# ysymyth/3D-SDN

Hardware: AMD Instinct MI355X
Metric: rendered-objects/sec (FFD decode + transform + silhouette/normal/depth @384, fwd+bwd) (higher is better)
Workload: dtype f32

## Files before the change

### 3d-sdn_amd/csrc/raster_fwd.hip

```cpp
#include <mutex>
#include <type_traits>
#include <vector>

#include "camera_math.h"
#include "raster_math.h"
#include "sdn_common.h"

namespace sdn {

constexpr int TS = 32;
constexpr int NTHR = (TS / 2) * (TS / 2);
constexpr int NWAVE = NTHR / 64;
static_assert(NTHR % 64 == 0 && NTHR >= 2 * TS && TS <= 32, "tile / workgroup geometry (hit queue packs px, py in 5 bits)");
constexpr int QCAP = 512;
constexpr int FREC = 13;
#ifndef SDN_LAB_FLAT_MAX
#define SDN_LAB_FLAT_MAX 256
#endif
constexpr int FLAT_MAX = SDN_LAB_FLAT_MAX;
static_assert(FLAT_MAX >= 1 && FLAT_MAX <= 256, "a batch's stream holds at most 64 * 256 candidates: 14 bits of start, at most 256 passes (the marks are u16, 0xffff = none)");
#ifndef SDN_LAB_HIZ_MIN_LIST
#define SDN_LAB_HIZ_MIN_LIST 257
#endif
constexpr int HIZ_MIN_LIST = SDN_LAB_HIZ_MIN_LIST;
#ifndef SDN_K1_HIZ
#define SDN_K1_HIZ 1
#endif
constexpr uint32_t TB_CULLED = 0x000000FFu;

struct FwdParams {
    const float* faces;
    const float* textures;
    const float* bg;
    float* face_inv;
    int32_t* face_index_map;
    float* weight_map;
    float* depth_map;
    float* rgb_map;
    float* rgb_out;
    float* alpha_out;
    float* depth_out;
    const uint32_t* tilebox;
    const uint4* pixbox;
    const uint32_t* tile_off;
    const uint32_t* tile_list;
    const uint32_t* overflow;
    const uint32_t* tile_order;
    const uint32_t* thin_count;
    const float4* thin_list;
    unsigned long long* counters;
    uint32_t list_cap;
    double eps;
    int ts, bs, nf, S, ntx, flags, bg_per_batch;
    int hiz;
    float near_le, far_f;
};

constexpr float THIN_MARGIN = 4.0f;

__device__ __forceinline__ float face_margin_px(const float f[9], int S)
{
    const float ex0 = f[3] - f[0], ey0 = f[4] - f[1];
    const float ex1 = f[6] - f[0], ey1 = f[7] - f[1];
    const float ex2 = f[6] - f[3], ey2 = f[7] - f[4];
    const float l0 = sqrtf(ex0 * ex0 + ey0 * ey0);
    const float l1 = sqrtf(ex1 * ex1 + ey1 * ey1);
    const float l2 = sqrtf(ex2 * ex2 + ey2 * ey2);
    const float lmax = fmaxf(l0, fmaxf(l1, l2));
    const float perim = l0 + l1 + l2;
    float cmax = fmaxf(fmaxf(fabsf(f[0]), fabsf(f[1])), fmaxf(fabsf(f[3]), fabsf(f[4])));
    cmax = fmaxf(cmax, fmaxf(fabsf(f[6]), fabsf(f[7])));
    const float area2 = fabsf(ex0 * ey1 - ex1 * ey0) - 9.5367432e-7f * lmax * lmax;
    if (!(area2 > 0.0f)) return -1.0f;
    const float delta = 9.5367432e-7f * (1.0f + cmax);
    const float base = 0.004f * fmaxf(1.0f, (float)S * (1.0f / 1024.0f)) + 0.5f * (float)S * delta;
    const float m = base + 0.5f * (float)S * (delta * perim * lmax / area2);
    if (!(m < (float)S)) return -1.0f;
    return m;
}

constexpr int HIST_MAX = 4096;

template <bool K1, bool GATHER>
__global__ __launch_bounds__(256) void k_face_setup(const float* __restrict__ faces, int nf, int S, int ntx,
                                                     float* __restrict__ face_inv, uint32_t* __restrict__ tilebox,
                                                     uint4* __restrict__ pixbox, uint32_t* __restrict__ tile_count,
                                                     uint32_t* __restrict__ thin_count, float4* __restrict__ thin_list,
                                                     const FaceSource G)
{
    __shared__ uint32_t hist[HIST_MAX];
    const int ntiles = ntx * ntx;
    const bool use_lds = ntiles <= HIST_MAX;
    if (use_lds)
        for (int t = threadIdx.x; t < ntiles; t += 256) hist[t] = 0u;
    __syncthreads();
    const int b = blockIdx.y;
    const int t_local = blockIdx.x * 256 + threadIdx.x;
    uint32_t* gcount = tile_count + (size_t)b * ntiles;
    const bool pairs = GATHER && G.fill_back != 0;
    const int nthr = pairs ? G.nf0 : nf;
    float v[3][3], pf[9];
    if constexpr (GATHER) {
        if (t_local < nthr) {
            const int32_t* idx = G.faces_idx + (size_t)b * G.fstride + (size_t)t_local * 3;
#pragma unroll
            for (int k = 0; k < 3; k++) {
                const float* p = G.verts + ((size_t)b * G.nv + idx[k]) * 3;
                v[k][0] = G.flip_x ? p[0] * -1.0f : p[0];
                v[k][1] = p[1];
                v[k][2] = p[2];
            }
            Basis B;
            if (G.mode != 0) B = camera_basis(G.mode, G.eye, G.dir, G.up, b);
            const float wv = G.width ? G.width[b] : 1.0f;
#pragma unroll
            for (int k = 0; k < 3; k++) {
                float o[3];
                project_vertex(v[k], G.mode, B, G.width != nullptr, wv, o);
                pf[3 * k + 0] = o[0];
                pf[3 * k + 1] = o[1];
                pf[3 * k + 2] = o[2];
            }
        }
    }
    if (t_local < nthr)
    for (int rep = 0; rep < (pairs ? 2 : 1); rep++) {
    const int fn_local = t_local + (rep ? G.nf0 : 0);
    const long i = (long)b * nf + fn_local;
    float f[9];
    float nrm[3] = {0.f, 0.f, 0.f};
    if constexpr (GATHER) {
        if (G.normals_out) {
            if (rep)
                face_normal(v[2], v[1], v[0], G.sx, nrm);
            else
                face_normal(v[0], v[1], v[2], G.sx, nrm);
        }
#pragma unroll
        for (int k = 0; k < 3; k++)
#pragma unroll
            for (int d = 0; d < 3; d++) f[3 * k + d] = rep ? pf[3 * (2 - k) + d] : pf[3 * k + d];
    } else {
#pragma unroll
        for (int k = 0; k < 9; k++) f[k] = faces[i * 9 + k];
    }
    float inv[9] = {0, 0, 0, 0, 0, 0, 0, 0, 0};
    uint32_t tb = TB_CULLED;
    uint4 pb = make_uint4(0, 0, 0, 0);
    bool thin = false;
    if constexpr (K1) {
      if (!is_backface(f)) {
        bool finite = true;
#pragma unroll
        for (int k = 0; k < 9; k++) finite = finite && (f[k] - f[k] == 0.0f);
        const K1Face K = k1_setup(f, S);
        if (finite && !K.dead && K.xi_min <= K.xi_max) {
            float inv_s[9];
            face_inverse(K.px, K.py, inv_s);
#pragma unroll
            for (int l = 0; l < 3; l++)
#pragma unroll
                for (int k = 0; k < 3; k++) {
                    const float v = inv_s[3 * l + k];
                    if (K.pi[l] == 0) inv[k] = v;
                    if (K.pi[l] == 1) inv[3 + k] = v;
                    if (K.pi[l] == 2) inv[6 + k] = v;
                }
            const float ymin = fminf(K.py[0], fminf(K.py[1], K.py[2])), ymax = fmaxf(K.py[0], fmaxf(K.py[1], K.py[2]));
            int y0 = 0, y1 = S - 1;
            if (!(K.px[2] < 0.0f)) {
                y0 = (int)fmaxf(floorf(ymin) - 1.0f, 0.0f);
                y1 = (int)fminf(ceilf(ymax) + 1.0f, (float)(S - 1));
            }
            if (y0 <= y1 && ymax + 1.0f >= 0.0f && ymin - 1.0f <= (float)(S - 1)) {
                const int x0 = K.xi_min, x1 = K.xi_max;
                tb = (uint32_t)(x0 / TS) | ((uint32_t)(x1 / TS) << 8) | ((uint32_t)(y0 / TS) << 16) | ((uint32_t)(y1 / TS) << 24);
                pb = make_uint4((uint32_t)x0 | ((uint32_t)x1 << 16), (uint32_t)y0 | ((uint32_t)y1 << 16), 0u, 0u);
                for (int ty = y0 / TS; ty <= y1 / TS; ty++)
                    for (int tx = x0 / TS; tx <= x1 / TS; tx++) {
                        if (use_lds)
                            atomicAdd(&hist[ty * ntx + tx], 1u);
                        else
                            atomicAdd(&gcount[ty * ntx + tx], 1u);
                    }
            }
        }
      }
    } else if (!is_backface(f)) {
        const float is_f = (float)S;
        float px[3], py[3];
#pragma unroll
        for (int k = 0; k < 3; k++) {
            px[k] = ndc_to_pixel(f[3 * k + 0], is_f);
            py[k] = ndc_to_pixel(f[3 * k + 1], is_f);
        }
        face_inverse(px, py, inv);
        int x0 = 0, x1 = S - 1, y0 = 0, y1 = S - 1;
        const float m = face_margin_px(f, S);
        const float xmin = fminf(px[0], fminf(px[1], px[2])), xmax = fmaxf(px[0], fmaxf(px[1], px[2]));
        const float ymin = fminf(py[0], fminf(py[1], py[2])), ymax = fmaxf(py[0], fmaxf(py[1], py[2]));
        const bool finite = (xmin - xmin == 0.0f) && (xmax - xmax == 0.0f) && (ymin - ymin == 0.0f) &&
                            (ymax - ymax == 0.0f) && (px[0] == px[0]) && (px[1] == px[1]) && (px[2] == px[2]) &&
                            (py[0] == py[0]) && (py[1] == py[1]) && (py[2] == py[2]);
        bool visible = true;
        if (!finite) {
            visible = false;
        } else if (!(m > 0.0f) || m > THIN_MARGIN) {
            visible = false;
            int ia = 0, ib = 1;
            float l2 = (px[1] - px[0]) * (px[1] - px[0]) + (py[1] - py[0]) * (py[1] - py[0]);
            const float l2b = (px[2] - px[0]) * (px[2] - px[0]) + (py[2] - py[0]) * (py[2] - py[0]);
            const float l2c = (px[2] - px[1]) * (px[2] - px[1]) + (py[2] - py[1]) * (py[2] - py[1]);
            if (l2b > l2) { l2 = l2b; ia = 0; ib = 2; }
            if (l2c > l2) { l2 = l2c; ia = 1; ib = 2; }
            if (l2 > 0.0f) {
                const float L = sqrtf(l2);
                const float nx = -(py[ib] - py[ia]) / L, ny = (px[ib] - px[ia]) / L;
                const int ic = 3 - ia - ib;
                const float h = fabsf((px[ic] - px[ia]) * nx + (py[ic] - py[ia]) * ny);
                const float pmax = fmaxf(fmaxf(fabsf(xmin), fabsf(xmax)), fmaxf(fabsf(ymin), fabsf(ymax)));
                float cmax = fmaxf(fmaxf(fabsf(f[0]), fabsf(f[1])), fmaxf(fabsf(f[3]), fabsf(f[4])));
                cmax = fmaxf(cmax, fmaxf(fabsf(f[6]), fabsf(f[7])));
                const float delta_px = 9.5367432e-7f * (1.0f + cmax) * 0.5f * (float)S;
                const float band = h + 0.05f + 2.5f * delta_px + 4e-6f * (pmax + (float)S);
                const bool repeated = (__float_as_uint(f[0]) == __float_as_uint(f[3]) && __float_as_uint(f[1]) == __float_as_uint(f[4])) ||
                                      (__float_as_uint(f[0]) == __float_as_uint(f[6]) && __float_as_uint(f[1]) == __float_as_uint(f[7])) ||
                                      (__float_as_uint(f[3]) == __float_as_uint(f[6]) && __float_as_uint(f[4]) == __float_as_uint(f[7]));
                int bx0 = 0, bx1 = S - 1, by0 = 0, by1 = S - 1;
                bool boxed_out = false;
                if (m > 0.0f) {
                    const float fx0 = ceilf(xmin - m), fx1 = floorf(xmax + m);
                    const float fy0 = ceilf(ymin - m), fy1 = floorf(ymax + m);
                    if (fx1 < 0.0f || fy1 < 0.0f || fx0 > (float)(S - 1) || fy0 > (float)(S - 1) || fx0 > fx1 || fy0 > fy1) {
                        boxed_out = true;
                    } else {
                        bx0 = (int)fmaxf(fx0, 0.0f);
                        by0 = (int)fmaxf(fy0, 0.0f);
                        bx1 = (int)fminf(fx1, (float)(S - 1));
                        by1 = (int)fminf(fy1, (float)(S - 1));
                    }
                }
                if (!(repeated && band < 0.5f) && !boxed_out) {
                    const uint32_t trange = (uint32_t)(bx0 / TS) | ((uint32_t)(bx1 / TS) << 8) | ((uint32_t)(by0 / TS) << 16) |
                                            ((uint32_t)(by1 / TS) << 24);
                    pb = make_uint4((uint32_t)bx0 | ((uint32_t)bx1 << 16), (uint32_t)by0 | ((uint32_t)by1 << 16), __float_as_uint(m), 0u);
                    const uint32_t slot = atomicAdd(&thin_count[b], 1u);
                    float4* e = thin_list + (size_t)b * nf * 2;
                    e[slot] = make_float4(nx, ny, px[ia] * nx + py[ia] * ny, band);
                    e[nf + slot] = make_float4(px[ia], py[ia], __uint_as_float((uint32_t)fn_local), __uint_as_float(trange));
                    thin = true;
                }
            }
        } else {
            const float fx0 = ceilf(xmin - m), fx1 = floorf(xmax + m);
            const float fy0 = ceilf(ymin - m), fy1 = floorf(ymax + m);
            if (fx1 < 0.0f || fy1 < 0.0f || fx0 > (float)(S - 1) || fy0 > (float)(S - 1) || fx0 > fx1 || fy0 > fy1) {
                visible = false;
            } else {
                x0 = (int)fmaxf(fx0, 0.0f);
                y0 = (int)fmaxf(fy0, 0.0f);
                x1 = (int)fminf(fx1, (float)(S - 1));
                y1 = (int)fminf(fy1, (float)(S - 1));
            }
        }
        if (visible) {
            tb = (uint32_t)(x0 / TS) | ((uint32_t)(x1 / TS) << 8) | ((uint32_t)(y0 / TS) << 16) |
                 ((uint32_t)(y1 / TS) << 24);
            pb = make_uint4((uint32_t)x0 | ((uint32_t)x1 << 16), (uint32_t)y0 | ((uint32_t)y1 << 16), __float_as_uint(m), 0u);
            for (int ty = y0 / TS; ty <= y1 / TS; ty++)
                for (int tx = x0 / TS; tx <= x1 / TS; tx++) {
                    if (use_lds)
                        atomicAdd(&hist[ty * ntx + tx], 1u);
                    else
                        atomicAdd(&gcount[ty * ntx + tx], 1u);
                }
        }
    }
    tilebox[i] = tb;
    if (!GATHER || tb != TB_CULLED || thin) {
#pragma unroll
        for (int k = 0; k < 9; k++) face_inv[i * 9 + k] = inv[k];
        pixbox[i] = pb;
        if constexpr (GATHER) {
            float* fo = G.faces_out + i * 9;
#pragma unroll
            for (int k = 0; k < 9; k++) fo[k] = f[k];
            if (G.normals_out) {
                float* o = G.normals_out + i * 3;
                o[0] = nrm[0];
                o[1] = nrm[1];
                o[2] = nrm[2];
            }
        }
    }
    }
    __syncthreads();
    if (use_lds)
        for (int t = threadIdx.x; t < ntiles; t += 256) {
            const uint32_t c = hist[t];
            if (c) atomicAdd(&gcount[t], c);
        }
}

constexpr int ORDER_CLASSES = 64;
__device__ __forceinline__ int order_class(uint32_t entries, bool streams_all_faces)
{
    if (streams_all_faces) return 0;
    const int c = (int)(4.0f * __log2f((float)entries + 1.0f));
    return ORDER_CLASSES - 1 - min(ORDER_CLASSES - 1, c);
}

__global__ __launch_bounds__(256) void k_tile_offsets(const uint32_t* __restrict__ tile_count, int ntiles,
                                                       uint32_t list_cap, uint32_t* __restrict__ tile_off,
                                                       uint32_t* __restrict__ overflow, uint32_t* __restrict__ order_hist)
{
    __shared__ uint32_t wave_tot[4];
    __shared__ uint32_t carry_s;
    __shared__ uint32_t hist[ORDER_CLASSES];
    const int b = blockIdx.x, tid = threadIdx.x;
    if (tid < ORDER_CLASSES) hist[tid] = 0u;
    const uint32_t* cnt = tile_count + (size_t)b * ntiles;
    uint32_t* off = tile_off + (size_t)b * (ntiles + 1);
    if (tid == 0) carry_s = 0u;
// ... 128 lines not shown
    float bgc[3] = {0.f, 0.f, 0.f};
    if (want_rgb) {
        const float* c = P.bg + (P.bg_per_batch ? 3 * b : 0);
        bgc[0] = c[0];
        bgc[1] = c[1];
        bgc[2] = c[2];
    }
    if (key == ~0ull) {
        r.fn = -1;
        r.w[0] = r.w[1] = r.w[2] = 0.0f;
        r.zp = P.far_f;
        r.alpha = 0.0f;
#pragma unroll
        for (int k = 0; k < 3; k++) r.rgb[k] = 0.0f * 0.0f + (1.0f - 0.0f) * bgc[k];
        return r;
    }
    const int fn = (int)(uint32_t)(key & 0xffffffffull);
    const size_t fidx = (size_t)b * P.nf + fn;
    float inv[9], f[9];
#pragma unroll
    for (int k = 0; k < 9; k++) inv[k] = P.face_inv[fidx * 9 + k];
#pragma unroll
    for (int k = 0; k < 9; k++) f[k] = P.faces[fidx * 9 + k];
    r.fn = fn;
    if (P.flags & SDN_K1_COVERAGE) {
        int pi[3];
        k1_order(f, pi);
        float inv_s[9], ws[3];
#pragma unroll
        for (int l = 0; l < 3; l++)
#pragma unroll
            for (int k = 0; k < 3; k++) inv_s[3 * l + k] = pi[l] == 0 ? inv[k] : (pi[l] == 1 ? inv[3 + k] : inv[6 + k]);
        bary_weights(inv_s, gx, gy, ws);
#pragma unroll
        for (int l = 0; l < 3; l++) {
            if (pi[l] == 0) r.w[0] = ws[l];
            if (pi[l] == 1) r.w[1] = ws[l];
            if (pi[l] == 2) r.w[2] = ws[l];
        }
    } else {
        bary_weights(inv, gx, gy, r.w);
    }
    r.zp = ord_unbits((uint32_t)(key >> 32));
    r.alpha = 1.0f;
    r.rgb[0] = r.rgb[1] = r.rgb[2] = 0.0f;
    if (want_rgb) {
        const bool face_color = (P.flags & SDN_FACE_COLOR) != 0;
        const int ts = face_color ? 2 : P.ts;
        const TexCoord tc = texture_coord(r.w, r.zp, f[2], f[5], f[8], ts, P.eps);
        const float* tex = face_color ? (P.textures + fidx * 3) : (P.textures + fidx * (size_t)ts * ts * ts * 3);
        float acc[3] = {0.f, 0.f, 0.f};
#pragma unroll
        for (int pn = 0; pn < 8; pn++) {
            int isc;
            float wgt;
            texture_corner(tc, pn, ts, isc, wgt);
            const float* t = face_color ? tex : (tex + (long)isc * 3);
#pragma unroll
            for (int k = 0; k < 3; k++) acc[k] = acc[k] + wgt * t[k];
        }
#pragma unroll
        for (int k = 0; k < 3; k++) r.rgb[k] = acc[k] * 1.0f + (1.0f - 1.0f) * bgc[k];
    }
    return r;
}

__device__ __forceinline__ void tile_epilogue(const FwdParams& P, const int b, const int X0, const int Y0,
                                              const unsigned long long* zbuf, const int tid)
{
    const int S = P.S;
    const bool aa = (P.flags & SDN_AA) != 0;
    const bool save = (P.flags & SDN_SAVE_MAPS) != 0;
    const bool lazy = (P.flags & SDN_LAZY_MAPS) != 0;
    const bool want_rgb = (P.flags & SDN_RGB) != 0;
    const bool want_alpha = (P.flags & SDN_ALPHA) != 0;
    const bool want_depth = (P.flags & SDN_DEPTH) != 0;
    const int qx = tid % (TS / 2), qy = tid / (TS / 2);
    const int R = aa ? S / 2 : S;
    float s_alpha = 0.f, s_depth = 0.f, s_rgb[3] = {0.f, 0.f, 0.f};
    bool any_valid = false;
#pragma unroll
    for (int dyi = 0; dyi < 2; dyi++) {
#pragma unroll
        for (int dx = 0; dx < 2; dx++) {
            const int dy = 1 - dyi;
            const int px = 2 * qx + dx, py = 2 * qy + dy;
            const int gx = X0 + px, gy = Y0 + py;
            if (gx >= S || gy >= S) continue;
            any_valid = true;
            const PixelResult r = shade_pixel(P, b, zbuf[py * TS + px], gx, gy);
            const size_t q = ((size_t)b * S + gy) * S + gx;
            if (save) {
                P.face_index_map[q] = r.fn;
                P.depth_map[q] = r.zp;
            }
            if (save && !lazy) {
                P.weight_map[q * 3 + 0] = r.w[0];
                P.weight_map[q * 3 + 1] = r.w[1];
                P.weight_map[q * 3 + 2] = r.w[2];
                if (want_rgb) {
                    P.rgb_map[q * 3 + 0] = r.rgb[0];
                    P.rgb_map[q * 3 + 1] = r.rgb[1];
                    P.rgb_map[q * 3 + 2] = r.rgb[2];
                }
            }
            if (aa) {
                s_alpha = s_alpha + r.alpha;
                s_depth = s_depth + r.zp;
#pragma unroll
                for (int k = 0; k < 3; k++) s_rgb[k] = s_rgb[k] + r.rgb[k];
            } else {
                const size_t o = ((size_t)b * S + (S - 1 - gy)) * S + gx;
                if (want_alpha) P.alpha_out[o] = r.alpha;
                if (want_depth) P.depth_out[o] = r.zp;
                if (want_rgb) {
#pragma unroll
                    for (int k = 0; k < 3; k++)
                        P.rgb_out[(((size_t)b * 3 + k) * S + (S - 1 - gy)) * S + gx] = r.rgb[k];
                }
            }
        }
    }
    if (aa && any_valid) {
        const int oc = X0 / 2 + qx;
        const int orow = R - 1 - (Y0 / 2 + qy);
        const size_t o = ((size_t)b * R + orow) * R + oc;
        if (want_alpha) P.alpha_out[o] = s_alpha * 0.25f;
        if (want_depth) P.depth_out[o] = s_depth * 0.25f;
        if (want_rgb) {
#pragma unroll
            for (int k = 0; k < 3; k++) P.rgb_out[(((size_t)b * 3 + k) * R + orow) * R + oc] = s_rgb[k] * 0.25f;
        }
    }
}

__device__ __forceinline__ void hiz_refresh(const uint32_t* zhi, uint32_t* blockmax, const int lane)
{
    uint32_t m[4] = {0u, 0u, 0u, 0u};
#pragma unroll
    for (int i = 0; i < 16; i++) m[i >> 2] = max(m[i >> 2], zhi[2 * (i * 64 + lane) + 1]);
#pragma unroll
    for (int rb = 0; rb < 4; rb++) {
        uint32_t v = m[rb];
        v = max(v, (uint32_t)__shfl_xor((int)v, 1, 64));
        v = max(v, (uint32_t)__shfl_xor((int)v, 2, 64));
        v = max(v, (uint32_t)__shfl_xor((int)v, 4, 64));
        v = max(v, (uint32_t)__shfl_xor((int)v, 32, 64));
        m[rb] = v;
    }
    if ((lane & 39) == 0) {
#pragma unroll
        for (int rb = 0; rb < 4; rb++) blockmax[rb * 4 + (lane >> 3)] = m[rb];
    }
    __builtin_amdgcn_wave_barrier();
}
__device__ __forceinline__ bool hiz_hidden(const uint32_t* blockmax, const uint32_t zc, const int x0, const int x1, const int y0,
                                           const int y1)
{
    uint32_t zb = 0u;
    for (int by = y0 >> 3; by <= (y1 >> 3); by++)
        for (int bx = x0 >> 3; bx <= (x1 >> 3); bx++) zb = max(zb, blockmax[by * (TS / 8) + bx]);
    return zc > zb;
}

template <bool COUNT, int HIZ>
__global__ __launch_bounds__(NTHR, 6) void k_raster_tiles(const FwdParams P)
{
    unsigned n_cand = 0, n_in = 0, n_key = 0;
    unsigned long long c_fetch = 0, c_small = 0, c_large = 0, c_thin = 0, c_epi = 0, t_mark = 0, t_begin = 0;
    auto tick = [&](unsigned long long& acc) {
        if constexpr (COUNT) {
            const unsigned long long now = wall_clock64();
            acc += now - t_mark;
            t_mark = now;
        }
    };
    if constexpr (COUNT) t_begin = t_mark = wall_clock64();
    __shared__ unsigned long long zbuf[TS * TS];
    __shared__ uint32_t q_fn[QCAP];
    __shared__ float xtab[TS], ytab[TS];
    __shared__ uint32_t q_count, next_batch, next_thin;
    __shared__ uint32_t hit_queue[NWAVE][128];
    __shared__ float face_rec[NWAVE][64 * FREC];
    __shared__ uint32_t blockmax[(TS / 8) * (TS / 8)];
    __shared__ uint32_t own_strip[NWAVE][32];
    static_assert(TS == 32, "the hi-z refresh maps 64 lanes x 16 reads onto a 32 x 32 tile");

    const int tid = threadIdx.x;
    const int lane = tid & 63, wave = tid >> 6;
    const int ntiles_all = P.ntx * P.ntx;
    const uint32_t gid = P.tile_order[blockIdx.x];
    const int b = (int)(gid / (uint32_t)ntiles_all), tile = (int)(gid % (uint32_t)ntiles_all);
    const int tx = tile % P.ntx, ty = tile / P.ntx;
    const int X0 = tx * TS, Y0 = ty * TS;
    const int S = P.S, nf = P.nf;

    for (int i = tid; i < TS * TS; i += NTHR) zbuf[i] = ~0ull;
    if (tid < TS)
        xtab[tid] = pixel_to_ndc(X0 + tid, S);
    else if (tid < 2 * TS)
        ytab[tid - TS] = pixel_to_ndc(Y0 + tid - TS, S);
    if (tid == 0) q_count = next_batch = next_thin = 0;
    if (tid < (TS / 8) * (TS / 8)) blockmax[tid] = 0xffffffffu;
    __syncthreads();

    const float4* thin_cull = P.thin_list + (size_t)b * nf * 2;
    const uint32_t n_thin = P.thin_count[b];
    const float4 thin_c0 = thin_cull[min(tid, 2 * nf - 1)];
    const uint32_t thin_r0 = reinterpret_cast<const uint32_t*>(thin_cull + nf + min(tid, nf - 1))[3];
    const uint32_t* tb = P.tilebox + (size_t)b * nf;
    const uint4* pbx = P.pixbox + (size_t)b * nf;
    const float* faces_b = P.faces + (size_t)b * nf * 9;
    const float* finv_b = P.face_inv + (size_t)b * nf * 9;

    auto shade_hit = [&](const float z0, const float z1, const float z2, const float (&inv)[9], const uint32_t qf,
                         const int px, const int py) {
        float bw[3];
        bary_weights(inv, X0 + px, Y0 + py, bw);
        const float zp = persp_depth(bw, z0, z1, z2);
        if (zp > P.near_le && zp < P.far_f) {
            if constexpr (COUNT) n_key++;
            const unsigned long long key = ((unsigned long long)ord_bits(zp) << 32) | qf;
            atomicMin(&zbuf[py * TS + px], key);
        }
    };
    uint32_t* hq = hit_queue[wave];
    float* frec = face_rec[wave];
    int hq_n = 0;
    auto drain = [&](const int count) {
        if (lane < count) {
            const uint32_t e = hq[lane];
            const int slot = (int)(e & 63u), px = (int)((e >> 6) & 31u), py = (int)((e >> 11) & 31u);
            const float* r = frec + slot * FREC;
            float inv[9];
#pragma unroll
            for (int k = 0; k < 9; k++) inv[k] = r[3 + k];
            shade_hit(r[0], r[1], r[2], inv, __float_as_uint(r[12]), px, py);
        }
    };
    const uint32_t* zhi = reinterpret_cast<const uint32_t*>(zbuf);
    auto behind = [&](const uint32_t zc, const int px, const int py) -> bool { return zc > zhi[2 * (py * TS + px) + 1]; };
    bool hiz_on = false;
    auto refresh_hiz = [&]() { hiz_refresh(zhi, blockmax, lane); };
    auto push_hits = [&](const bool hit, const uint32_t entry) {
        const unsigned long long hm = __ballot(hit);
        if (hm) {
            if (hit) hq[hq_n + (int)__popcll(hm & ((1ull << lane) - 1ull))] = entry;
            hq_n += (int)__popcll(hm);
            __builtin_amdgcn_wave_barrier();
            if (hq_n >= 64) {
                drain(64);
                __builtin_amdgcn_wave_barrier();
                const uint32_t rest = (lane < hq_n - 64) ? hq[64 + lane] : 0u;
                __builtin_amdgcn_wave_barrier();
                hq[lane] = rest;
                hq_n -= 64;
                __builtin_amdgcn_wave_barrier();
            }
        }
    };
    auto raster_batch = [&](const uint32_t* ids, const int n) {
        if constexpr (HIZ > 0) {
            if (HIZ == 1 || hiz_on) refresh_hiz();
        }
        const bool mine = lane < n;
        const uint32_t qf_l = mine ? ids[lane] : 0u;
        uint4 pb_l = make_uint4(0u, 0u, 0u, 0u);
        float f_l[9], inv_l[9];
#pragma unroll
        for (int kk = 0; kk < 9; kk++) f_l[kk] = inv_l[kk] = 0.0f;
        if (mine) {
            pb_l = pbx[qf_l];
#pragma unroll
            for (int kk = 0; kk < 9; kk++) f_l[kk] = faces_b[(size_t)qf_l * 9 + kk];
#pragma unroll
            for (int kk = 0; kk < 9; kk++) inv_l[kk] = finv_b[(size_t)qf_l * 9 + kk];
        }
        const int lx0 = max((int)(pb_l.x & 0xffffu), X0), lx1 = min((int)(pb_l.x >> 16), X0 + TS - 1);
        const int ly0 = max((int)(pb_l.y & 0xffffu), Y0), ly1 = min((int)(pb_l.y >> 16), Y0 + TS - 1);
        const int lw = lx1 - lx0 + 1, lh = ly1 - ly0 + 1;
        int area_l = (mine && lw > 0 && lh > 0) ? lw * lh : 0;
        const float zmin_l = fminf(f_l[2], fminf(f_l[5], f_l[8]));
        const uint32_t zc_l = (zmin_l > 0.0f) ? ord_bits(zmin_l * 0.99999f) : 0u;
        if constexpr (HIZ > 0) {
            if ((HIZ == 1 || hiz_on) && area_l > 0 && zc_l != 0u && hiz_hidden(blockmax, zc_l, lx0 - X0, lx1 - X0, ly0 - Y0, ly1 - Y0))
                area_l = 0;
        }
        if (mine) {
            float* r = frec + lane * FREC;
            r[0] = f_l[2];
            r[1] = f_l[5];
            r[2] = f_l[8];
#pragma unroll
            for (int kk = 0; kk < 9; kk++) r[3 + kk] = inv_l[kk];
            r[12] = __uint_as_float(qf_l);
        }
        __builtin_amdgcn_wave_barrier();
        if constexpr (COUNT) {
            asm volatile("s_waitcnt vmcnt(0) lgkmcnt(0)" ::: "memory");
            tick(c_fetch);
        }
        unsigned long long big = __ballot(area_l > FLAT_MAX);
        {
            const int fa = area_l <= FLAT_MAX ? area_l : 0;
            int incl = fa;
#pragma unroll
            for (int d = 1; d < 64; d <<= 1) {
                const int o = __shfl_up(incl, d, 64);
                if (lane >= d) incl += o;
            }
            const int T = __builtin_amdgcn_readlane(incl, 63);
            const int box_l = ((lx0 - X0) & 31) | (((ly0 - Y0) & 31) << 5) | (((lw - 1) & 31) << 10) | ((incl - fa) << 15) |
                              (fa > 0 ? 0 : (int)0x80000000);
            const float rw_l = 1.0f / (float)(lw > 0 ? lw : 1);
            const unsigned long long fm = __ballot(fa > 0);
            const int below = (int)__builtin_amdgcn_mbcnt_hi((uint32_t)(fm >> 32), __builtin_amdgcn_mbcnt_lo((uint32_t)fm, 0u));
            const int rank_l = fa > 0 ? below : (int)__popcll(fm) + lane - below;
            const int lane_of_rank = __builtin_amdgcn_ds_permute(rank_l << 2, lane);
            uint32_t* strip = own_strip[wave];
            uint16_t* strip16 = reinterpret_cast<uint16_t*>(strip);
            if (lane < 32) strip[lane] = 0xffffffffu;
            __builtin_amdgcn_wave_barrier();
            int rank0 = -1;
            for (int base = 0, pass = 0; base < T; base += 64, pass++) {
                const int rel = (box_l >> 15) - base;
                if ((unsigned)rel < 64u) strip16[rel] = (uint16_t)pass;
                __builtin_amdgcn_wave_barrier();
                const bool starts = (int)strip16[lane] == pass;
                __builtin_amdgcn_wave_barrier();
                const unsigned long long sm = __ballot(starts);
                const int rk = (int)__builtin_amdgcn_mbcnt_hi((uint32_t)(sm >> 32),
                                                              __builtin_amdgcn_mbcnt_lo((uint32_t)sm, (uint32_t)(rank0 + (starts ? 1 : 0))));
                rank0 += (int)__popcll(sm);
                const int s = __builtin_amdgcn_ds_bpermute(rk << 2, lane_of_rank);
                const int a4 = s << 2;
                const int box = __builtin_amdgcn_ds_bpermute(a4, box_l);
                const float rw = __int_as_float(__builtin_amdgcn_ds_bpermute(a4, __float_as_int(rw_l)));
                const uint32_t zc = (uint32_t)__builtin_amdgcn_ds_bpermute(a4, (int)zc_l);
                float f[9];
#pragma unroll
                for (int kk = 0; kk < 9; kk++)
                    f[kk] = (kk % 3 == 2) ? 0.0f : __int_as_float(__builtin_amdgcn_ds_bpermute(a4, __float_as_int(f_l[kk])));
                bool hit = false;
                int px = 0, py = 0;
                if (base + lane < T) {
                    const int i = base + lane - (box >> 15);
                    const int yy = (int)(((float)i + 0.5f) * rw);
                    const int xx = i - yy * (((box >> 10) & 31) + 1);
                    px = (box & 31) + xx;
                    py = ((box >> 5) & 31) + yy;
                    if constexpr (COUNT) n_cand++;
                    hit = inside_ndc(f, xtab[px], ytab[py]);
                    if constexpr (COUNT) n_in += hit ? 1u : 0u;
                    if (hit) hit = !behind(zc, px, py);
                }
                push_hits(hit, (uint32_t)s | ((uint32_t)px << 6) | ((uint32_t)py << 11));
            }
        }
        tick(c_small);
        const float fS = (float)S, fS1 = (float)(S - 1);
        while (big) {
            const int j = __builtin_amdgcn_readfirstlane(__ffsll((long long)big) - 1);
            big &= big - 1ull;
            const uint32_t pbx_j = (uint32_t)__builtin_amdgcn_readlane((int)pb_l.x, j), pby_j = (uint32_t)__builtin_amdgcn_readlane((int)pb_l.y, j);
            const int x0 = max((int)(pbx_j & 0xffffu), X0), y0 = max((int)(pby_j & 0xffffu), Y0);
            const int w = min((int)(pbx_j >> 16), X0 + TS - 1) - x0 + 1, h = min((int)(pby_j >> 16), Y0 + TS - 1) - y0 + 1;
            const uint32_t zc = (uint32_t)__builtin_amdgcn_readlane((int)zc_l, j);
            const float mj = __int_as_float(__builtin_amdgcn_readlane((int)pb_l.z, j));
            const uint32_t slot = (uint32_t)j;
            float f[9];
#pragma unroll
            for (int kk = 0; kk < 9; kk++) f[kk] = __int_as_float(__builtin_amdgcn_readlane(__float_as_int(f_l[kk]), j));
            const int hs = h > 1 ? 32 - __clz(h - 1) : 0;
            const int rshift = 6 - hs, per_row = 1 << rshift;
            const int row = lane >> rshift, rsub = lane & (per_row - 1);
            const bool rvalid = row < h;
            const int py = y0 - Y0 + (rvalid ? row : 0);
            const float yp = ytab[py];
            const int bx0 = x0 - X0;
            float lo = (float)bx0, hi = (float)(bx0 + w - 1);
#pragma unroll
            for (int e = 0; e < 3; e++) {
                const float xa = f[3 * e], ya = f[3 * e + 1], xb = f[(3 * e + 3) % 9], yb = f[(3 * e + 4) % 9];
                const float D = xb - xa, E = yb - ya;
                if (E != 0.0f) {
                    const float rE = __builtin_amdgcn_rcpf(E);
                    const float xe = xa + (yp - ya) * D * rE;
                    const float pe = (xe * fS + fS1) * 0.5f - (float)X0;
                    const float sl = mj * __builtin_amdgcn_sqrtf(D * D + E * E) * fabsf(rE) + 1.0f;
                    if (E > 0.0f)
                        hi = fminf(hi, pe + sl);
                    else
                        lo = fmaxf(lo, pe - sl);
                }
            }
            const int xl = max(bx0, (int)floorf(fminf(lo, 64.0f)));
            const int xr = min(bx0 + w - 1, (int)ceilf(fmaxf(hi, -64.0f)));
            const int len = rvalid ? xr - xl + 1 : 0;
            for (int i = rsub; __ballot(i < len) != 0ull; i += per_row) {
                bool hit = false;
                int px = 0;
                if (i < len) {
                    px = xl + i;
                    if constexpr (COUNT) n_cand++;
                    hit = inside_ndc(f, xtab[px], yp);
                    if constexpr (COUNT) n_in += hit ? 1u : 0u;
                    if (hit) hit = !behind(zc, px, py);
                }
                push_hits(hit, slot | ((uint32_t)px << 6) | ((uint32_t)py << 11));
            }
        }
        if (hq_n) {
            drain(hq_n);
            hq_n = 0;
            __builtin_amdgcn_wave_barrier();
        }
        tick(c_large);
    };

    const float4* thin_recs = thin_cull + nf;
    auto thin_cull_pass = [&]() {
        const float cx = (float)X0 + 0.5f * (float)(TS - 1), cy = (float)Y0 + 0.5f * (float)(TS - 1);
        const float reach = 0.7072f * (float)TS + 0.4f;
#ifndef SDN_LAB_NO_THIN_CULL
        for (uint32_t t = tid; t < n_thin; t += NTHR) {
            const float4 c = t < (uint32_t)NTHR ? thin_c0 : thin_cull[t];
            if (fabsf(cx * c.x + cy * c.y - c.z) > c.w + reach) continue;
            const uint32_t v = t < (uint32_t)NTHR ? thin_r0 : reinterpret_cast<const uint32_t*>(thin_recs + t)[3];
            if ((uint32_t)tx < (v & 255u) || (uint32_t)tx > ((v >> 8) & 255u) || (uint32_t)ty < ((v >> 16) & 255u) || (uint32_t)ty > (v >> 24)) continue;
            const uint32_t slot = atomicAdd(&q_count, 1u);
            if (slot < (uint32_t)QCAP) q_fn[slot] = t;
        }
#endif
    };
    auto thin_items = [&]() {
#ifndef SDN_LAB_NO_THIN
        const uint32_t queued = q_count;
        const bool all = queued > (uint32_t)QCAP;
        const uint32_t n_loop = all ? n_thin : queued;
        constexpr int ROWS_PER_ITEM = 8, GROUPS = TS / ROWS_PER_ITEM;
        for (;;) {
            uint32_t first = 0;
            if (lane == 0) first = atomicAdd(&next_thin, 64u);
            first = (uint32_t)__builtin_amdgcn_readfirstlane((int)first);
            if (first >= n_loop * GROUPS) break;
            const uint32_t item = first + (uint32_t)lane;
            if (item >= n_loop * GROUPS) continue;
            const uint32_t c = item / GROUPS;
            const int g = (int)(item % GROUPS);
            const uint32_t t = all ? c : q_fn[c];
            const float4 e0 = thin_cull[t], e1 = thin_recs[t];
            const float nx = e0.x, ny = e0.y, band = e0.w, ax = e1.x, ay = e1.y;
            const uint32_t qf = __float_as_uint(e1.z);
            const uint4 pbq = pbx[qf];
            const int cx0 = max((int)(pbq.x & 0xffffu) - X0, 0), cx1 = min((int)(pbq.x >> 16) - X0, TS - 1);
            const int cy0 = max((int)(pbq.y & 0xffffu) - Y0, g * ROWS_PER_ITEM), cy1 = min((int)(pbq.y >> 16) - Y0, (g + 1) * ROWS_PER_ITEM - 1);
            if (cx0 > cx1) continue;
            float f[9];
            bool loaded = false;
            for (int py = cy0; py <= cy1; py++) {
                const float off = ((float)(Y0 + py) - ay) * ny;
                int lo = cx0, hi = cx1;
                if (fabsf(nx) > 1e-3f) {
                    const float r = 1.0f / nx;
                    const float xa = ax + (-band - off) * r, xb = ax + (band - off) * r;
                    const float x_lo = fminf(xa, xb) - (float)X0 - 1.0f, x_hi = fmaxf(xa, xb) - (float)X0 + 1.0f;
                    if (!(x_lo <= (float)(TS - 1)) || !(x_hi >= 0.0f)) continue;
                    lo = max(cx0, (int)fmaxf(x_lo, 0.0f));
                    hi = min(cx1, (int)fminf(x_hi, (float)(TS - 1)));
                } else if (fabsf(off + ((float)X0 + 0.5f * (float)(TS - 1) - ax) * nx) > band + 0.5f * (float)TS * fabsf(nx) + 1.0f) {
                    continue;
                }
                for (int px = lo; px <= hi; px++) {
                    const float dist = fabsf(((float)(X0 + px) - ax) * nx + ((float)(Y0 + py) - ay) * ny);
                    if (!(dist <= band)) continue;
                    if (!loaded) {
#pragma unroll
                        for (int k = 0; k < 9; k++) f[k] = faces_b[(size_t)qf * 9 + k];
                        loaded = true;
                    }
                    if (inside_ndc(f, xtab[px], ytab[py])) {
                        float inv[9];
#pragma unroll
                        for (int k = 0; k < 9; k++) inv[k] = finv_b[(size_t)qf * 9 + k];
                        float w[3];
                        bary_weights(inv, X0 + px, Y0 + py, w);
                        const float zp = persp_depth(w, f[2], f[5], f[8]);
                        if (zp > P.near_le && zp < P.far_f) {
                            const unsigned long long key = ((unsigned long long)ord_bits(zp) << 32) | qf;
                            atomicMin(&zbuf[py * TS + px], key);
                        }
                    }
                }
            }
        }
#endif
    };

    if (P.overflow[b] == 0u) {
        const int ntiles = P.ntx * P.ntx;
        const uint32_t* off = P.tile_off + (size_t)b * (ntiles + 1);
        const uint32_t lo = off[tile], hi = off[tile + 1];
        tick(c_fetch);
        thin_cull_pass();
        __syncthreads();
        tick(c_thin);
        const uint32_t* lst = P.tile_list + (size_t)b * P.list_cap + lo;
        const int n_list = (int)(hi - lo);
        hiz_on = n_list >= HIZ_MIN_LIST;
        if (n_list <= 64 * NWAVE) {
            const int per_wave = (n_list + NWAVE - 1) / NWAVE;
            const int run_lo = wave * per_wave, run_hi = min(n_list, run_lo + per_wave);
            if (run_lo < run_hi) raster_batch(lst + run_lo, run_hi - run_lo);
        } else {
            for (;;) {
                int base = 0;
                if (lane == 0) base = (int)atomicAdd(&next_batch, 64u);
                base = __builtin_amdgcn_readfirstlane(base);
                if (base >= n_list) break;
                raster_batch(lst + base, min(64, n_list - base));
            }
        }
        thin_items();
        tick(c_thin);
    } else {
        for (int base = 0; base < nf; base += NTHR) {
            const int fn = base + tid;
            if (fn < nf) {
                const uint32_t v = tb[fn];
                const bool hit = (uint32_t)tx >= (v & 255u) && (uint32_t)tx <= ((v >> 8) & 255u) &&
                                 (uint32_t)ty >= ((v >> 16) & 255u) && (uint32_t)ty <= (v >> 24);
                if (hit) {
                    const uint32_t slot = atomicAdd(&q_count, 1u);
                    q_fn[slot] = (uint32_t)fn;
                }
            }
            __syncthreads();
            const int cnt = (int)q_count;
            __syncthreads();
            const bool last = base + NTHR >= nf;
            if (cnt >= NTHR || (last && cnt > 0)) {
                const int per_wave = (cnt + NWAVE - 1) / NWAVE;
                const int run_lo = wave * per_wave, run_hi = min(cnt, run_lo + per_wave);
                for (int qb = run_lo; qb < run_hi; qb += 64) raster_batch(q_fn + qb, min(64, run_hi - qb));
                __syncthreads();
                if (tid == 0) q_count = 0;
                __syncthreads();
            }
        }
        thin_cull_pass();
        __syncthreads();
        thin_items();
    }
    __syncthreads();
    tick(c_fetch);


    tile_epilogue(P, b, X0, Y0, zbuf, tid);
    if constexpr (COUNT) {
        tick(c_epi);
        __shared__ unsigned long long cnt[3];
        if (tid < 3) cnt[tid] = 0ull;
        __syncthreads();
        unsigned long long c[3] = {n_cand, n_in, n_key};
#pragma unroll
        for (int k = 0; k < 3; k++) {
#pragma unroll
            for (int o = 32; o > 0; o >>= 1) c[k] += __shfl_xor(c[k], o, 64);
            if (lane == 0 && c[k]) atomicAdd(&cnt[k], c[k]);
        }
        __syncthreads();
        if (tid < 3 && cnt[tid]) atomicAdd(P.counters + tid, cnt[tid]);
        if (lane == 0 && (gid & 15u) == 0u) {
            atomicAdd(P.counters + 3, c_fetch);
            atomicAdd(P.counters + 4, c_small);
            atomicAdd(P.counters + 5, c_large);
            atomicAdd(P.counters + 6, c_thin);
            atomicAdd(P.counters + 7, c_epi);
            atomicAdd(P.counters + 8, t_mark - t_begin);
            atomicMax(P.counters + 9, t_mark - t_begin);
            atomicAdd(P.counters + 10, 1ull);
        }
    }
}

__global__ __launch_bounds__(NTHR) void k_raster_tiles_k1(const FwdParams P)
{
    __shared__ unsigned long long zbuf[TS * TS];
    __shared__ uint32_t next_batch;
    __shared__ uint32_t hit_queue[NWAVE][128];
    __shared__ float face_rec[NWAVE][64 * FREC];
    __shared__ uint32_t blockmax[(TS / 8) * (TS / 8)];
    bool hiz_on = false;
    const int tid = threadIdx.x;
    const int lane = tid & 63, wave = tid >> 6;
    const int ntiles = P.ntx * P.ntx;
    const uint32_t gid = P.tile_order[blockIdx.x];
    const int b = (int)(gid / (uint32_t)ntiles), tile = (int)(gid % (uint32_t)ntiles);
    const int tx = tile % P.ntx, ty = tile / P.ntx;
    const int X0 = tx * TS, Y0 = ty * TS;
    const int S = P.S, nf = P.nf;
    for (int i = tid; i < TS * TS; i += NTHR) zbuf[i] = ~0ull;
    if (tid == 0) next_batch = 0;
    if (tid < (TS / 8) * (TS / 8)) blockmax[tid] = 0xffffffffu;
    __syncthreads();
    const uint4* pbx = P.pixbox + (size_t)b * nf;
    const uint32_t* tb = P.tilebox + (size_t)b * nf;
    const float* faces_b = P.faces + (size_t)b * nf * 9;
    const float* finv_b = P.face_inv + (size_t)b * nf * 9;
    const uint32_t* zhi = reinterpret_cast<const uint32_t*>(zbuf);
    uint32_t* hq = hit_queue[wave];
    float* frec = face_rec[wave];
    int hq_n = 0;
    auto drain = [&](const int count) {
        if (lane < count) {
            const uint32_t e = hq[lane];
            const int slot = (int)(e & 63u), px = (int)((e >> 6) & 31u), py = (int)((e >> 11) & 31u);
            const float* r = frec + slot * FREC;
            float inv_s[9], w[3];
#pragma unroll
            for (int k = 0; k < 9; k++) inv_s[k] = r[3 + k];
            bary_weights(inv_s, X0 + px, Y0 + py, w);
            const float zp = persp_depth(w, r[0], r[1], r[2]);
            if (zp > P.near_le && zp < P.far_f) {
                const unsigned long long key = ((unsigned long long)ord_bits(zp) << 32) | __float_as_uint(r[12]);
                atomicMin(&zbuf[py * TS + px], key);
            }
        }
    };
    auto behind = [&](const uint32_t zc, const int px, const int py) -> bool { return zc > zhi[2 * (py * TS + px) + 1]; };
    auto push_hits = [&](const bool hit, const uint32_t entry) {
        const unsigned long long hm = __ballot(hit);
        if (hm) {
            if (hit) hq[hq_n + (int)__popcll(hm & ((1ull << lane) - 1ull))] = entry;
            hq_n += (int)__popcll(hm);
            __builtin_amdgcn_wave_barrier();
            if (hq_n >= 64) {
                drain(64);
                __builtin_amdgcn_wave_barrier();
                const uint32_t rest = (lane < hq_n - 64) ? hq[64 + lane] : 0u;
                __builtin_amdgcn_wave_barrier();
                hq[lane] = rest;
                hq_n -= 64;
                __builtin_amdgcn_wave_barrier();
            }
        }
    };
    constexpr int K1_SMALL = 32;
    auto raster_batch = [&](const bool have, const uint32_t fn) {
        if (hiz_on && SDN_K1_HIZ) hiz_refresh(zhi, blockmax, lane);
        float f[9], inv[9];
#pragma unroll
        for (int k = 0; k < 9; k++) f[k] = inv[k] = 0.0f;
        uint4 pb = make_uint4(0u, 0u, 0u, 0u);
        if (have) {
#pragma unroll
            for (int k = 0; k < 9; k++) f[k] = faces_b[(size_t)fn * 9 + k];
#pragma unroll
            for (int k = 0; k < 9; k++) inv[k] = finv_b[(size_t)fn * 9 + k];
// ... 523 lines not shown
```

### 3d-sdn_amd/csrc/raster_math.h

```cpp
#pragma once
#include <hip/hip_runtime.h>
#include <stdint.h>

namespace sdn {

__device__ __forceinline__ int cvt_i32(float v)
{
    if (v != v) return 0;
    if (v >= 2147483648.0f) return 2147483647;
    if (v <= -2147483648.0f) return (int)0x80000000;
    return (int)v;
}

__device__ __forceinline__ bool is_backface(const float f[9])
{
    const float a = (f[7] - f[1]) * (f[3] - f[0]);
    const float b = (f[4] - f[1]) * (f[6] - f[0]);
    return a < b;
}

__device__ __forceinline__ float ndc_to_pixel(float v, float is_f)
{
    float t = v * is_f;
    t = t + is_f;
    t = t - 1.0f;
    return 0.5f * t;
}

__device__ __forceinline__ float pixel_to_ndc(int i, int is)
{
    return (float)((2. * (double)i + 1. - (double)is) / (double)is);
}

__device__ __forceinline__ float face_inverse(const float px[3], const float py[3], float inv[9])
{
    inv[0] = py[1] - py[2];
    inv[1] = px[2] - px[1];
    inv[2] = px[1] * py[2] - px[2] * py[1];
    inv[3] = py[2] - py[0];
    inv[4] = px[0] - px[2];
    inv[5] = px[2] * py[0] - px[0] * py[2];
    inv[6] = py[0] - py[1];
    inv[7] = px[1] - px[0];
    inv[8] = px[0] * py[1] - px[1] * py[0];
    float den = px[2] * (py[0] - py[1]) + px[0] * (py[1] - py[2]);
    den = den + px[1] * (py[2] - py[0]);
#pragma unroll
    for (int k = 0; k < 9; k++) inv[k] = inv[k] / den;
    return den;
}

__device__ __forceinline__ bool inside_ndc(const float f[9], float xp, float yp)
{
    if ((yp - f[1]) * (f[3] - f[0]) < (xp - f[0]) * (f[4] - f[1])) return false;
    if ((yp - f[4]) * (f[6] - f[3]) < (xp - f[3]) * (f[7] - f[4])) return false;
    if ((yp - f[7]) * (f[0] - f[6]) < (xp - f[6]) * (f[1] - f[7])) return false;
    return true;
}

__device__ __forceinline__ void bary_weights(const float inv[9], int xi, int yi, float w[3])
{
    const float fx = (float)xi, fy = (float)yi;
    float sum = 0.0f;
#pragma unroll
    for (int k = 0; k < 3; k++) {
        float t = inv[3 * k + 0] * fx + inv[3 * k + 1] * fy;
        t = t + inv[3 * k + 2];
        t = fminf(fmaxf(t, 0.0f), 1.0f);
        w[k] = t;
        sum = sum + t;
    }
#pragma unroll
    for (int k = 0; k < 3; k++) w[k] = w[k] / sum;
}

__device__ __forceinline__ float persp_depth(const float w[3], float z0, float z1, float z2)
{
    float s = w[0] / z0 + w[1] / z1;
    s = s + w[2] / z2;
    return 1.0f / s;
}

__device__ __forceinline__ int cvt_i32_d(double v)
{
    if (v != v) return 0;
    if (v >= 2147483647.0) return 2147483647;
    if (v <= -2147483648.0) return (int)0x80000000;
    return (int)v;
}

struct K1Face {
    float px[3], py[3];
    float sa, sb, sc;
    int pi[3];
    int xi_min, xi_max;
    bool a_ok, b_ok, dead;
};

__device__ __forceinline__ void k1_order(const float f[9], int pi[3])
{
    if (f[0] < f[3]) {
        pi[0] = (f[6] < f[0]) ? 2 : 0;
        pi[2] = (f[3] < f[6]) ? 2 : 1;
    } else {
        pi[0] = (f[6] < f[3]) ? 2 : 1;
        pi[2] = (f[0] < f[6]) ? 2 : 0;
    }
    pi[1] = 0;
#pragma unroll
    for (int k = 0; k < 3; k++)
        if (pi[0] != k && pi[2] != k) pi[1] = k;
}

__device__ __forceinline__ K1Face k1_setup(const float f[9], int is)
{
    K1Face K;
    k1_order(f, K.pi);
    const float is_f = (float)is;
#pragma unroll
    for (int l = 0; l < 3; l++) {
        const int k = K.pi[l];
        const float x = k == 0 ? f[0] : (k == 1 ? f[3] : f[6]);
        const float y = k == 0 ? f[1] : (k == 1 ? f[4] : f[7]);
        K.px[l] = ndc_to_pixel(x, is_f);
        K.py[l] = ndc_to_pixel(y, is_f);
    }
    K.dead = K.px[0] == K.px[2];
    K.a_ok = K.px[1] - K.px[0] != 0.0f;
    K.b_ok = K.px[2] - K.px[1] != 0.0f;
    K.sa = (K.py[1] - K.py[0]) / (K.px[1] - K.px[0]);
    K.sb = (K.py[2] - K.py[1]) / (K.px[2] - K.px[1]);
    K.sc = (K.py[2] - K.py[0]) / (K.px[2] - K.px[0]);
    K.xi_min = cvt_i32_d(fmax((double)ceilf(K.px[0]), 0.));
    K.xi_max = cvt_i32_d(fmin((double)K.px[2], (double)is - 1.));
    return K;
}

__device__ __forceinline__ void k1_column(const K1Face& K, int xi, int is, int& yi_min, int& yi_max)
{
    yi_min = 0;
    yi_max = -1;
    if (xi < K.xi_min || xi > K.xi_max) return;
    const float fx = (float)xi;
    float yi1;
    if (fx <= K.px[1]) {
        float s = K.sa * (fx - K.px[0]);
        yi1 = K.a_ok ? s + K.py[0] : K.py[1];
    } else {
        float s = K.sb * (fx - K.px[1]);
        yi1 = K.b_ok ? s + K.py[1] : K.py[1];
    }
    float s2 = K.sc * (fx - K.px[0]);
    const float yi2 = s2 + K.py[0];
    yi_min = cvt_i32_d(fmax(0., (double)ceilf(fminf(yi1, yi2))));
    yi_max = cvt_i32_d(fmin((double)fmaxf(yi1, yi2), (double)is - 1.));
}

__device__ __forceinline__ uint32_t ord_bits(float v)
{
    const uint32_t b = __float_as_uint(v);
    return (b & 0x80000000u) ? ~b : (b | 0x80000000u);
}
__device__ __forceinline__ float ord_unbits(uint32_t o)
{
    const uint32_t b = (o & 0x80000000u) ? (o & 0x7fffffffu) : ~o;
    return __uint_as_float(b);
}

struct TexCoord {
    int base[3];
    float frac[3];
};

__device__ __forceinline__ TexCoord texture_coord(const float w[3], float depth, float z0, float z1, float z2,
                                                  int ts, double eps)
{
    TexCoord tc;
    const float z[3] = {z0, z1, z2};
    const double c = (double)(ts - 1) - eps;
#pragma unroll
    for (int k = 0; k < 3; k++) {
        const float q = depth / z[k];
        const float tif = (float)(((double)w[k] * c) * (double)q);
        const int b = cvt_i32(tif);
        tc.base[k] = b;
        tc.frac[k] = tif - (float)b;
    }
    return tc;
}

__device__ __forceinline__ void texture_corner(const TexCoord& tc, int pn, int ts, int& isc, float& wgt)
{
    float w = 1.0f;
    int idx[3];
#pragma unroll
    for (int k = 0; k < 3; k++) {
        if (((pn >> k) & 1) == 0) {
            w = w * (1.0f - tc.frac[k]);
            idx[k] = tc.base[k];
        } else {
            w = w * tc.frac[k];
            idx[k] = tc.base[k] + 1;
        }
    }
    isc = idx[0] * ts * ts + idx[1] * ts + idx[2];
    wgt = w;
}

}
```

Before: 25290.

## Stream small-face candidates as runs of four pixels per lane

In the small-face rasterization stream, each lane now handles a run of up to four horizontally adjacent pixels rather than one pixel. The y-dependent part of the edge tests is computed once per row and reused for every pixel in the run. This cuts the number of candidate slots, stream passes and bpermute broadcasts per face. The cost is extra inner-loop work per lane, wasted slots when a box width is not a multiple of the run length, and more push_hits calls per pass. It also reads the depth buffer directly in place of the behind() helper.

```diff
diff --git a/3d-sdn_amd/csrc/raster_fwd.hip b/3d-sdn_amd/csrc/raster_fwd.hip
--- a/3d-sdn_amd/csrc/raster_fwd.hip
+++ b/3d-sdn_amd/csrc/raster_fwd.hip
@@ -19,6 +19,12 @@
 #endif
 constexpr int FLAT_MAX = SDN_LAB_FLAT_MAX;
 static_assert(FLAT_MAX >= 1 && FLAT_MAX <= 256, "a batch's stream holds at most 64 * 256 candidates: 14 bits of start, at most 256 passes (the marks are u16, 0xffff = none)");
+#ifndef SDN_LAB_STREAM_GROUP
+#define SDN_LAB_STREAM_GROUP 4
+#endif
+constexpr int STREAM_G = SDN_LAB_STREAM_GROUP;
+static_assert(STREAM_G == 1 || STREAM_G == 2 || STREAM_G == 4, "a run is 1, 2 or 4 pixels (its column count is a shift of the box width)");
+constexpr int STREAM_SH = STREAM_G == 4 ? 2 : STREAM_G == 2 ? 1 : 0;
 #ifndef SDN_LAB_HIZ_MIN_LIST
 #define SDN_LAB_HIZ_MIN_LIST 257
 #endif
@@ -753,7 +759,8 @@
         }
         unsigned long long big = __ballot(area_l > FLAT_MAX);
         {
-            const int fa = area_l <= FLAT_MAX ? area_l : 0;
+            const int gw_l = ((lw > 0 ? lw : 1) + STREAM_G - 1) >> STREAM_SH;
+            const int fa = (area_l > 0 && area_l <= FLAT_MAX) ? gw_l * lh : 0;
             int incl = fa;
 #pragma unroll
             for (int d = 1; d < 64; d <<= 1) {
@@ -763,7 +770,7 @@
             const int T = __builtin_amdgcn_readlane(incl, 63);
             const int box_l = ((lx0 - X0) & 31) | (((ly0 - Y0) & 31) << 5) | (((lw - 1) & 31) << 10) | ((incl - fa) << 15) |
                               (fa > 0 ? 0 : (int)0x80000000);
-            const float rw_l = 1.0f / (float)(lw > 0 ? lw : 1);
+            const float rw_l = 1.0f / (float)gw_l;
             const unsigned long long fm = __ballot(fa > 0);
             const int below = (int)__builtin_amdgcn_mbcnt_hi((uint32_t)(fm >> 32), __builtin_amdgcn_mbcnt_lo((uint32_t)fm, 0u));
             const int rank_l = fa > 0 ? below : (int)__popcll(fm) + lane - below;
@@ -792,20 +799,35 @@
 #pragma unroll
                 for (int kk = 0; kk < 9; kk++)
                     f[kk] = (kk % 3 == 2) ? 0.0f : __int_as_float(__builtin_amdgcn_ds_bpermute(a4, __float_as_int(f_l[kk])));
-                bool hit = false;
-                int px = 0, py = 0;
+                uint32_t e0 = (uint32_t)s;
+                int left = 0;
+                float lhs[3] = {0.0f, 0.0f, 0.0f}, dy[3] = {0.0f, 0.0f, 0.0f};
                 if (base + lane < T) {
+                    const int lwm1 = (box >> 10) & 31;
+                    const int gw = (lwm1 >> STREAM_SH) + 1;
                     const int i = base + lane - (box >> 15);
                     const int yy = (int)(((float)i + 0.5f) * rw);
-                    const int xx = i - yy * (((box >> 10) & 31) + 1);
-                    px = (box & 31) + xx;
-                    py = ((box >> 5) & 31) + yy;
-                    if constexpr (COUNT) n_cand++;
-                    hit = inside_ndc(f, xtab[px], ytab[py]);
-                    if constexpr (COUNT) n_in += hit ? 1u : 0u;
-                    if (hit) hit = !behind(zc, px, py);
+                    const int xx = (i - yy * gw) << STREAM_SH;
+                    const int px0 = (box & 31) + xx;
+                    const int py = ((box >> 5) & 31) + yy;
+                    left = lwm1 + 1 - xx;
+                    e0 |= ((uint32_t)px0 << 6) | ((uint32_t)py << 11);
+                    inside_ndc_row(f, ytab[py], lhs, dy);
                 }
-                push_hits(hit, (uint32_t)s | ((uint32_t)px << 6) | ((uint32_t)py << 11));
+                const int pidx = (int)(e0 >> 6);
+                bool hit[STREAM_G];
+#pragma unroll
+                for (int j = 0; j < STREAM_G; j++) {
+                    hit[j] = false;
+                    if (j < left) {
+                        if constexpr (COUNT) n_cand++;
+                        hit[j] = inside_ndc_px(f, lhs, dy, xtab[(pidx & 31) + j]);
+                        if constexpr (COUNT) n_in += hit[j] ? 1u : 0u;
+                        if (hit[j]) hit[j] = !(zc > zhi[2 * (pidx + j) + 1]);
+                    }
+                }
+#pragma unroll
+                for (int j = 0; j < STREAM_G; j++) push_hits(hit[j], e0 + ((uint32_t)j << 6));
             }
         }
         tick(c_small);
diff --git a/3d-sdn_amd/csrc/raster_math.h b/3d-sdn_amd/csrc/raster_math.h
--- a/3d-sdn_amd/csrc/raster_math.h
+++ b/3d-sdn_amd/csrc/raster_math.h
@@ -58,6 +58,24 @@
     return true;
 }
 
+__device__ __forceinline__ void inside_ndc_row(const float f[9], float yp, float lhs[3], float dy[3])
+{
+    lhs[0] = (yp - f[1]) * (f[3] - f[0]);
+    lhs[1] = (yp - f[4]) * (f[6] - f[3]);
+    lhs[2] = (yp - f[7]) * (f[0] - f[6]);
+    dy[0] = f[4] - f[1];
+    dy[1] = f[7] - f[4];
+    dy[2] = f[1] - f[7];
+}
+
+__device__ __forceinline__ bool inside_ndc_px(const float f[9], const float lhs[3], const float dy[3], float xp)
+{
+    if (lhs[0] < (xp - f[0]) * dy[0]) return false;
+    if (lhs[1] < (xp - f[3]) * dy[1]) return false;
+    if (lhs[2] < (xp - f[6]) * dy[2]) return false;
+    return true;
+}
+
 __device__ __forceinline__ void bary_weights(const float inv[9], int xi, int yi, float w[3])
 {
     const float fx = (float)xi, fy = (float)yi;
```

Result: faster. 26010 (median of 6 runs) (+2.8%).
